# murongshaozong/fabric-token-sdk

Measured on AMD Instinct MI355X. Metric: range-proof verifies/sec (BN254, 64-bit), higher is better.
Workload: dtype u32 (BN254 Fp/Fr 8x32-bit Montgomery); 1 GPU; C2: batch of 4096 standalone 64-bit Bulletproof range proofs per GPU (exact transcripts per proof + RLC batch check via one Pippenger MSM); batch_per_gpu=4096, bit_length=64, rounds=6, parallelism=shard1

## Files before the change

### fabric-token-sdk_amd/csrc/device/fixed_base.hpp

```cpp
#pragma once
#include "g1.hpp"

namespace fts {

constexpr int FB_W = 16;
constexpr int FB_NW = (255 + FB_W - 1) / FB_W;
constexpr int FB_E = 1 << (FB_W - 1);
constexpr size_t FB_WORDS_PER_BASE = (size_t)FB_NW * FB_E * 16;
constexpr int FB_S = 1 << ((FB_W) / 2);
constexpr int FB_L = FB_E / FB_S;

template <int W>
struct FbCfg {
  static constexpr int NW = (255 + W - 1) / W;
  static constexpr int E = 1 << (W - 1);
  static constexpr size_t WORDS_PER_BASE = (size_t)NW * E * 16;
  static constexpr int S = 1 << (W / 2);
  static constexpr int L = E / S;
};
constexpr int FBW_W = 20;
using FbWide = FbCfg<FBW_W>;

FTS_DEV int fb_next_digit(uint32_t s[8], int& carry) {
  int d = (int)(s[0] & (uint32_t)(2 * FB_E - 1)) + carry;
// ... 2 lines not shown
  s[7] >>= FB_W;
  carry = d > FB_E;
  return carry ? d - 2 * FB_E : d;
}

FTS_DEV void madd_inl(G1J& p, const G1A& q) {
  if (f_is_zero(p.z)) {
    p.x = q.x;
    p.y = q.y;
    p.z = f_one<FpP>();
    return;
  }
  Fp z1z1 = fp_sqr(p.z);
  Fp u2 = fp_mul(q.x, z1z1);
  Fp s2 = fp_mul(fp_mul(q.y, p.z), z1z1);
  Fp h = f_sub(u2, p.x);
  Fp rr = f_sub(s2, p.y);
  if (f_is_zero(h)) {
    p = f_is_zero(rr) ? g1j_dbl(p) : g1j_identity();
    return;
  }
  Fp hh = fp_sqr(h);
  Fp i = f_dbl(f_dbl(hh));
  Fp j = fp_mul(h, i);
  rr = f_dbl(rr);
  Fp v = fp_mul(p.x, i);
  Fp x3 = f_sub(f_sub(fp_sqr(rr), j), f_dbl(v));
  Fp y3 = f_sub(fp_mul(rr, f_sub(v, x3)), f_dbl(fp_mul(p.y, j)));
  p.z = f_sub(f_sub(fp_sqr(f_add(p.z, h)), z1z1), hh);
  p.x = x3;
  p.y = y3;
}

FTS_DEV G1A fb_entry(const uint32_t* __restrict__ table, int w, int d) {
  const int ad = d < 0 ? -d : d;
  G1A q = load_g1a(table + ((size_t)w * FB_E + (ad - 1)) * 16);
  if (d < 0) q.y = f_neg(q.y);
  return q;
}

FTS_DEV G1J fb_mul(const uint32_t* __restrict__ table, const Scalar& k) {
  uint32_t s[8];
#pragma unroll
  for (int i = 0; i < 8; i++) s[i] = k.v[i];
  G1J acc = g1j_identity();
  int carry = 0, w = 0, d = 0;
  for (; w < FB_NW; w++) {
    d = fb_next_digit(s, carry);
    if (d != 0) break;
  }
  if (w == FB_NW) return acc;
  G1A cur = fb_entry(table, w, d);
  for (;;) {
    int wn = w + 1, dn = 0;
    for (; wn < FB_NW; wn++) {
      dn = fb_next_digit(s, carry);
      if (dn != 0) break;
    }
    G1A nxt;
    if (wn < FB_NW) nxt = fb_entry(table, wn, dn);
    madd_inl(acc, cur);
    if (wn >= FB_NW) break;
    cur = nxt;
    w = wn;
  }
  return acc;
}

FTS_DEV G1J fb_mul2(const uint32_t* __restrict__ ta, const Scalar& ka, const uint32_t* __restrict__ tb,
                    const Scalar& kb) {
  uint32_t sa[8], sb[8];
#pragma unroll
  for (int i = 0; i < 8; i++) sa[i] = ka.v[i], sb[i] = kb.v[i];
  G1J acc = g1j_identity();
  int ca = 0, cb = 0;
  int da = fb_next_digit(sa, ca), db = fb_next_digit(sb, cb);
  G1A qa, qb;
  if (da != 0) qa = fb_entry(ta, 0, da);
  if (db != 0) qb = fb_entry(tb, 0, db);
  for (int w = 0; w < FB_NW; w++) {
    int dan = 0, dbn = 0;
    G1A na, nb;
    if (w + 1 < FB_NW) {
      dan = fb_next_digit(sa, ca);
      dbn = fb_next_digit(sb, cb);
      if (dan != 0) na = fb_entry(ta, w + 1, dan);
      if (dbn != 0) nb = fb_entry(tb, w + 1, dbn);
    }
    if (da != 0) madd_inl(acc, qa);
    if (db != 0) madd_inl(acc, qb);
    da = dan, db = dbn, qa = na, qb = nb;
  }
  return acc;
}

template <int W>
FTS_DEV int fb_next_digit_w(uint32_t s[8], int& carry) {
  constexpr int E = FbCfg<W>::E;
  int d = (int)(s[0] & (uint32_t)(2 * E - 1)) + carry;
#pragma unroll
  for (int i = 0; i < 7; i++) s[i] = (s[i] >> W) | (s[i + 1] << (32 - W));
  s[7] >>= W;
  carry = d > E;
  return carry ? d - 2 * E : d;
}
template <int W>
FTS_DEV G1A fb_entry_w(const uint32_t* __restrict__ table, int w, int d) {
  const int ad = d < 0 ? -d : d;
  G1A q = load_g1a(table + ((size_t)w * FbCfg<W>::E + (ad - 1)) * 16);
  if (d < 0) q.y = f_neg(q.y);
  return q;
}
template <int W>
FTS_DEV G1J fb_mul_w(const uint32_t* __restrict__ table, const Scalar& k) {
  constexpr int NW = FbCfg<W>::NW;
  uint32_t s[8];
#pragma unroll
  for (int i = 0; i < 8; i++) s[i] = k.v[i];
  G1J acc = g1j_identity();
  int carry = 0, w = 0, d = 0;
  for (; w < NW; w++) {
    d = fb_next_digit_w<W>(s, carry);
    if (d != 0) break;
  }
  if (w == NW) return acc;
  G1A cur = fb_entry_w<W>(table, w, d);
  for (;;) {
    int wn = w + 1, dn = 0;
    for (; wn < NW; wn++) {
      dn = fb_next_digit_w<W>(s, carry);
      if (dn != 0) break;
    }
    G1A nxt;
    if (wn < NW) nxt = fb_entry_w<W>(table, wn, dn);
    madd_inl(acc, cur);
    if (wn >= NW) break;
    cur = nxt;
    w = wn;
  }
  return acc;
}

FTS_DEV void fb_mul_acc(G1J& acc, const uint32_t* __restrict__ table, const Scalar& k) {
  uint32_t s[8];
#pragma unroll
  for (int i = 0; i < 8; i++) s[i] = k.v[i];
  int carry = 0, w = 0, d = 0;
  for (; w < FB_NW; w++) {
    d = fb_next_digit(s, carry);
    if (d != 0) break;
  }
  if (w == FB_NW) return;
  G1A cur = fb_entry(table, w, d);
  for (;;) {
    int wn = w + 1, dn = 0;
    for (; wn < FB_NW; wn++) {
      dn = fb_next_digit(s, carry);
      if (dn != 0) break;
    }
    G1A nxt;
    if (wn < FB_NW) nxt = fb_entry(table, wn, dn);
    madd_inl(acc, cur);
    if (wn >= FB_NW) break;
    cur = nxt;
    w = wn;
  }
}

template <int W>
FTS_DEV void fb_mul_acc_w(G1J& acc, const uint32_t* __restrict__ table, const Scalar& k) {
  constexpr int NW = FbCfg<W>::NW;
  uint32_t s[8];
#pragma unroll
  for (int i = 0; i < 8; i++) s[i] = k.v[i];
  int carry = 0, w = 0, d = 0;
  for (; w < NW; w++) {
    d = fb_next_digit_w<W>(s, carry);
    if (d != 0) break;
  }
  if (w == NW) return;
  G1A cur = fb_entry_w<W>(table, w, d);
  for (;;) {
    int wn = w + 1, dn = 0;
    for (; wn < NW; wn++) {
      dn = fb_next_digit_w<W>(s, carry);
      if (dn != 0) break;
    }
    G1A nxt;
    if (wn < NW) nxt = fb_entry_w<W>(table, wn, dn);
    madd_inl(acc, cur);
    if (wn >= NW) break;
    cur = nxt;
    w = wn;
  }
}

__device__ __noinline__ G1J nl_fb_mul(const uint32_t* __restrict__ table, Scalar k) { return fb_mul(table, k); }

}
```

### fabric-token-sdk_amd/csrc/device/g1.hpp

```cpp
#pragma once
#include "field.hpp"

namespace fts {

struct G1A {
  Fp x, y;
};
struct G1J {
  Fp x, y, z;
};
struct Scalar {
  uint32_t v[8];
};

struct G1J;
__device__ __noinline__ G1J nl_dbl(G1J p);

FTS_DEV Fp fp_mul(const Fp& a, const Fp& b) { return f_mul_g(a, b); }
FTS_DEV Fp fp_sqr(const Fp& a) { return f_mul_g(a, a); }
FTS_DEV Fr fr_mul(const Fr& a, const Fr& b) { return f_mul_g(a, b); }
FTS_DEV Fr fr_sqr(const Fr& a) { return f_mul_g(a, a); }

FTS_DEV G1J g1j_identity() {
  G1J r;
// ... 63 lines not shown
  G1J r;
  r.x = f_sub(f_sub(fp_sqr(rr), j), f_dbl(v));
  r.y = f_sub(fp_mul(rr, f_sub(v, r.x)), f_dbl(fp_mul(p.y, j)));
  r.z = f_sub(f_sub(fp_sqr(f_add(p.z, h)), z1z1), hh);
  return r;
}

FTS_DEV G1J g1j_add(const G1J& p, const G1J& q) {
  if (f_is_zero(p.z)) return q;
  if (f_is_zero(q.z)) return p;
  Fp z1z1 = fp_sqr(p.z);
  Fp z2z2 = fp_sqr(q.z);
  Fp u1 = fp_mul(p.x, z2z2);
  Fp u2 = fp_mul(q.x, z1z1);
  Fp s1 = fp_mul(fp_mul(p.y, q.z), z2z2);
  Fp s2 = fp_mul(fp_mul(q.y, p.z), z1z1);
  Fp h = f_sub(u2, u1);
  Fp rr = f_sub(s2, s1);
  if (f_is_zero(h)) {
    if (f_is_zero(rr)) return nl_dbl(p);
    return g1j_identity();
  }
  Fp i = fp_sqr(f_dbl(h));
  Fp j = fp_mul(h, i);
  rr = f_dbl(rr);
  Fp v = fp_mul(u1, i);
  G1J r;
  r.x = f_sub(f_sub(fp_sqr(rr), j), f_dbl(v));
  r.y = f_sub(fp_mul(rr, f_sub(v, r.x)), f_dbl(fp_mul(s1, j)));
  r.z = fp_mul(f_sub(f_sub(fp_sqr(f_add(p.z, q.z)), z1z1), z2z2), h);
  return r;
}

__device__ __noinline__ Fp nl_fp_inv(Fp a) { return f_inv_gcd(a); }
__device__ __noinline__ Fr nl_fr_inv(Fr a) { return f_inv_gcd(a); }

FTS_DEV bool g1j_eq(const G1J& p, const G1J& q) {
  bool pi = f_is_zero(p.z), qi = f_is_zero(q.z);
  if (pi || qi) return pi && qi;
  Fp z1z1 = fp_sqr(p.z), z2z2 = fp_sqr(q.z);
  if (!f_eq(fp_mul(p.x, z2z2), fp_mul(q.x, z1z1))) return false;
  return f_eq(fp_mul(fp_mul(p.y, q.z), z2z2), fp_mul(fp_mul(q.y, p.z), z1z1));
}

FTS_DEV G1A g1j_to_affine(const G1J& p) {
  G1A r;
  if (f_is_zero(p.z)) {
    r.x = f_zero<FpP>();
    r.y = f_zero<FpP>();
    return r;
  }
  Fp zi = nl_fp_inv(p.z);
  Fp zi2 = fp_sqr(zi);
  r.x = fp_mul(p.x, zi2);
  r.y = fp_mul(fp_mul(p.y, zi2), zi);
  return r;
}

__device__ __noinline__ G1J nl_dbl(G1J p) { return g1j_dbl(p); }

FTS_DEV void load_fp(const uint32_t* src, Fp& a) {
  const uint4* s = reinterpret_cast<const uint4*>(src);
  uint4 u0 = s[0], u1 = s[1];
  a.v[0] = u0.x; a.v[1] = u0.y; a.v[2] = u0.z; a.v[3] = u0.w;
  a.v[4] = u1.x; a.v[5] = u1.y; a.v[6] = u1.z; a.v[7] = u1.w;
}
// ... 102 lines not shown
```

### fabric-token-sdk_amd/csrc/device/glv.hpp

```cpp
#pragma once
#include "fixed_base.hpp"

namespace fts {

struct Glv {
  static constexpr uint32_t BETA[8] = {0xd782e155u, 0x71930c11u, 0xffbe3323u, 0xa6bb947cu,
                                       0xd4741444u, 0xaa303344u, 0x26594943u, 0x2c3b3f0du};
  static constexpr uint32_t G1[7] = {0x2fafba64u, 0x8fa7d32du, 0x773a6ef2u, 0x6eb9c714u,
                                     0xc7e0b3d7u, 0xd91d232eu, 0x00000002u};
  static constexpr uint32_t G2[9] = {0x9b9bdffau, 0x86937516u, 0x5eaa26d9u, 0xa5e38cfbu, 0x391eb18du,
                                     0x7a7bd9d4u, 0xa773d2cfu, 0x4ccef014u, 0x00000002u};
  static constexpr uint32_t A1[2] = {0x94d213e3u, 0x89d32568u};
  static constexpr uint32_t A2[4] = {0x1221250bu, 0x0be4e154u, 0xeeb859fdu, 0x6f4d8248u};
  static constexpr uint32_t NB1[4] = {0x7d4f1128u, 0x8211bbebu, 0xeeb859fcu, 0x6f4d8248u};
};

template <int G>
FTS_DEV void glv_round(const uint32_t k[8], const uint32_t (&g)[G], uint32_t c[5]) {
  uint32_t t[8 + G];
#pragma unroll
  for (int i = 0; i < 8 + G; i++) t[i] = 0;
#pragma unroll
  for (int i = 0; i < 8; i++) {
    uint64_t carry = 0;
// ... 46 lines not shown

template <class K = Glv>
FTS_DEV void glv_decompose(const uint32_t k[8], uint32_t k1[4], uint32_t& s1, uint32_t k2[4], uint32_t& s2) {
  uint32_t c1[5], c2[5];
  glv_round<7>(k, K::G1, c1);
  glv_round<9>(k, K::G2, c2);
  uint32_t r1[8], r2[8];
#pragma unroll
  for (int i = 0; i < 8; i++) {
    r1[i] = k[i];
    r2[i] = 0;
  }
  sub_mul_256<3, 2>(r1, c1, K::A1);
  sub_mul_256<5, 4>(r1, c2, K::A2);
  sub_mul_256<5, 2>(r2, c2, K::A1);
  {
    uint32_t p[8];
#pragma unroll
    for (int i = 0; i < 8; i++) p[i] = 0;
    sub_mul_256<3, 4>(p, c1, K::NB1);
    uint32_t bw = 0;
#pragma unroll
    for (int i = 0; i < 8; i++) r2[i] = subb(r2[i], p[i], bw, bw);
  }
  s1 = glv_abs(r1, k1);
  s2 = glv_abs(r2, k2);
}

FTS_DEV Fp glv_beta() {
  Fp b;
#pragma unroll
  for (int i = 0; i < 8; i++) b.v[i] = Glv::BETA[i];
  return b;
}

FTS_DEV void add_inl(G1J& p, const G1J& q) {
  if (f_is_zero(q.z)) return;
  if (f_is_zero(p.z)) {
    p = q;
    return;
  }
  Fp z1z1 = fp_sqr(p.z);
  Fp z2z2 = fp_sqr(q.z);
  Fp u1 = fp_mul(p.x, z2z2);
  Fp u2 = fp_mul(q.x, z1z1);
  Fp s1 = fp_mul(fp_mul(p.y, q.z), z2z2);
  Fp s2 = fp_mul(fp_mul(q.y, p.z), z1z1);
  Fp h = f_sub(u2, u1);
  Fp rr = f_sub(s2, s1);
  if (f_is_zero(h)) {
    p = f_is_zero(rr) ? g1j_dbl(p) : g1j_identity();
    return;
  }
  Fp i = fp_sqr(f_dbl(h));
  Fp j = fp_mul(h, i);
  rr = f_dbl(rr);
  Fp v = fp_mul(u1, i);
  Fp x3 = f_sub(f_sub(fp_sqr(rr), j), f_dbl(v));
  Fp y3 = f_sub(fp_mul(rr, f_sub(v, x3)), f_dbl(fp_mul(s1, j)));
  p.z = fp_mul(f_sub(f_sub(fp_sqr(f_add(p.z, q.z)), z1z1), z2z2), h);
  p.x = x3;
  p.y = y3;
}

FTS_DEV void vtab_store(uint32_t* __restrict__ tab, size_t stride, size_t idx, int e, const G1J& p) {
#pragma unroll
  for (int i = 0; i < 8; i++) {
    tab[((size_t)(e * 24) + i) * stride + idx] = p.x.v[i];
    tab[((size_t)(e * 24) + 8 + i) * stride + idx] = p.y.v[i];
    tab[((size_t)(e * 24) + 16 + i) * stride + idx] = p.z.v[i];
  }
}
FTS_DEV G1J vtab_load(const uint32_t* __restrict__ tab, size_t stride, size_t idx, int e) {
  G1J p;
#pragma unroll
  for (int i = 0; i < 8; i++) {
    p.x.v[i] = tab[((size_t)(e * 24) + i) * stride + idx];
    p.y.v[i] = tab[((size_t)(e * 24) + 8 + i) * stride + idx];
    p.z.v[i] = tab[((size_t)(e * 24) + 16 + i) * stride + idx];
  }
  return p;
}

FTS_DEV G1J vb128j(const G1J& t, const uint32_t kk[4], uint32_t* __restrict__ tab, size_t stride, size_t idx) {
  if (f_is_zero(t.z)) return g1j_identity();
  {
    vtab_store(tab, stride, idx, 0, t);
    G1J cur = g1j_dbl(t);
    vtab_store(tab, stride, idx, 1, cur);
    for (int e = 2; e < 8; e++) {
      add_inl(cur, t);
      vtab_store(tab, stride, idx, e, cur);
    }
  }
  uint32_t s[4];
// ... 328 lines not shown
```

### fabric-token-sdk_amd/csrc/device/rp_kernels.hpp

```cpp
#pragma once
#include <hip/hip_runtime.h>
#include <stdint.h>
#include "launch.hpp"

namespace fts {

constexpr int RP_PT_T1 = 0, RP_PT_T2 = 1, RP_PT_C = 2, RP_PT_D = 3, RP_PT_V = 4, RP_PT_L = 5;
inline __host__ __device__ int rp_npts(int k) { return 5 + 2 * k; }

constexpr int RP_SC_TAU = 0, RP_SC_DELTA = 1, RP_SC_IP = 2, RP_SC_A = 3, RP_SC_B = 4, RP_NSC = 5;

constexpr int CH_X = 0, CH_X2 = 1, CH_Y = 2, CH_YINV = 3, CH_Z = 4, CH_Z2 = 5, CH_POL = 6, CH_X0 = 7, CH_XJ = 8;
inline __host__ __device__ int rp_nch(int k) { return 8 + 2 * k; }

inline __host__ __device__ int tb_G(int n) { return 2 * n; }
inline __host__ __device__ int tb_H(int n) { return 2 * n + 1; }
inline __host__ __device__ int tb_P(int n) { return 2 * n + 2; }
inline __host__ __device__ int tb_Q(int n) { return 2 * n + 3; }
inline __host__ __device__ int tb_K(int n) { return 2 * n + 4; }
inline __host__ __device__ int tb_ped0(int n) { return 2 * n + 5; }
inline __host__ __device__ int tb_count(int n) { return 2 * n + 6; }

inline __host__ __device__ uint32_t x0_array_len(int n) { return 130u * (2u * n + 2u) - 2u; }
inline __host__ __device__ uint32_t x0_msg_len(int n) { return x0_array_len(n) + 46u; }
inline __host__ __device__ uint32_t x0_slot_bytes(int n) { return ((x0_msg_len(n) + 9u + 63u) / 64u) * 64u; }
inline __host__ __device__ uint32_t x0_const_off(int n) { return 8u + 130u * n; }
inline __host__ __device__ uint32_t x0_const_end(int n) { return 8u + 130u * (2u * n + 1u); }
inline __host__ __device__ uint32_t x0_cb0(int n) { return (x0_const_off(n) + 63u) / 64u; }
inline __host__ __device__ uint32_t x0_cb1(int n) { return x0_const_end(n) / 64u; }
inline __host__ __device__ uint32_t x0_var_bytes(int n) { return x0_slot_bytes(n) - 64u * (x0_cb1(n) - x0_cb0(n)); }

constexpr uint32_t SMALL_SLOT = 512;

constexpr double MADS_PER_MUL = 136.0;
constexpr double COST_MADD = 11.0;
constexpr double COST_ADD = 16.0;
constexpr double COST_DBL = 7.0;
constexpr double COST_INV = 0.0;
constexpr double COST_NORM1 = COST_INV + 4.0;
constexpr double COST_FB = 16.0 * COST_MADD;
constexpr double COST_FB_FRESH = 15.0 * COST_MADD;
constexpr double COST_FBW = 13.0 * COST_MADD;
constexpr double COST_FBW_FRESH = 12.0 * COST_MADD;
constexpr double COST_VB4 = 7.0 + 6.0 * COST_MADD + 256.0 * COST_DBL + 60.0 * COST_ADD;
constexpr double COST_VB128 = 7.0 + 6.0 * COST_ADD + 124.0 * COST_DBL + 30.0 * COST_ADD;
constexpr double COST_STRAUS2 = 2.0 * (7.0 + 6.0 * COST_ADD) + 124.0 * COST_DBL + 60.0 * COST_ADD;
constexpr double COST_STRAUS2_ATAB = (COST_DBL + 6.0 * COST_MADD) + (COST_DBL + 6.0 * COST_ADD) + 109.0 +
                                     124.0 * COST_DBL + 60.0 * COST_MADD;
constexpr double COST_STRAUS2_CTAB = (COST_DBL + 6.0 * COST_ADD) + 61.0 + 124.0 * COST_DBL + 60.0 * COST_MADD;
constexpr double COST_NORM = 7.0;

struct Timeline {
  static constexpr int CAP = 96;
  bool in_fallback = false;
  static constexpr int MAXS = 4;
  hipEvent_t ev[CAP + 1];
  const char* name[CAP];
  double work[CAP];
  int start[CAP];
  int n = 0;
  hipStream_t sl[MAXS];
  int last[MAXS];
  int ns = 0;
  bool created = false;
  void create() {
    if (created) return;
    for (int i = 0; i <= CAP; i++) (void)hipEventCreate(&ev[i]);
    created = true;
  }
  void destroy() {
    if (!created) return;
    for (int i = 0; i <= CAP; i++) (void)hipEventDestroy(ev[i]);
    created = false;
  }
  int& last_of(hipStream_t s) {
    for (int i = 0; i < ns; i++)
// ... 104 lines not shown
```

### fabric-token-sdk_amd/csrc/idemix_identity.hip

```cpp
#include <hip/hip_runtime.h>
#include <stdint.h>
#include <string.h>
#include <sys/random.h>

#include <algorithm>
#include <atomic>
#include <functional>
#include <memory>
#include <mutex>
#include <string>
#include <type_traits>
#include <unordered_map>
#include <vector>

#include "../../include/fts_gpu.h"
#include "common/chacha20.hpp"
#include "common/sha256.hpp"
#include "device/fixed_base.hpp"
#include "device/glv.hpp"
#include "device/helpers.hpp"
#include "device/transcript.hpp"
#include "device/fp256bn.hpp"
#include "device/pairing.hpp"
#include "device/launch.hpp"
// ... 34 lines not shown
  using PJ = G1J;
  static constexpr int G1_BYTES = 64;
  static FTS_DEV PJ inf() { return g1j_identity(); }
  static FTS_DEV bool is_inf(const PJ& p) { return f_is_zero(p.z); }
  static FTS_DEV PJ dbl(const PJ& p) { return g1j_dbl(p); }
  static FTS_DEV void add_to(PJ& acc, const PJ& q) { add_inl(acc, q); }
  static FTS_DEV void madd_to(PJ& acc, const F& x, const F& y) {
    G1A q;
    q.x = x, q.y = y;
    madd_inl(acc, q);
  }
  static FTS_DEV PJ from_affine(const F& x, const F& y) {
    PJ r;
    r.x = x, r.y = y, r.z = f_one<FpP>();
    return r;
  }
  static FTS_DEV bool decode(const uint8_t* raw, F& x, F& y, bool& ident) {
    G1A a;
    const bool ok = decode_point(raw, a);
    ident = ok && g1a_is_identity(a);
    x = a.x, y = a.y;
    return ok;
  }
  template <class Sink>
  static FTS_DEV void encode(Sink& s, const F& x, const F& y) {
    uint32_t pw[16];
    g1_mont_to_be_words(x, y, pw);
    for (int k = 0; k < 16; k++) s.put_word(pw[k]);
  }
  static FTS_DEV void fixed_mul_acc(PJ& acc, const uint32_t* tables, int base, const uint32_t* k) {
    Scalar s;
#pragma unroll
    for (int q = 0; q < 8; q++) s.v[q] = k[q];
    fb_mul_acc(acc, tables + (size_t)base * FB_WORDS_PER_BASE, s);
  }
  static FTS_DEV void decompose(const uint32_t k[8], uint32_t k1[4], uint32_t& s1, uint32_t k2[4], uint32_t& s2) {
    glv_decompose<Glv>(k, k1, s1, k2, s2);
  }
  static FTS_DEV F beta() { return glv_beta(); }
  static FTS_DEV void digest_mod_r(const uint32_t st[8], uint32_t out[8]) {
    const Fr r = digest_to_fr(st);
#pragma unroll
    for (int q = 0; q < 8; q++) out[q] = r.v[q];
  }
};

constexpr int FBN_NW = 16, FBN_ND = 1 << 16;
struct FbnCurve {
  using B = pair::FbnField;
  using F = fbn::Fp;
  using PJ = fbn::PJ;
  static constexpr int G1_BYTES = 65;
  static FTS_DEV PJ inf() { return fbn::pj_inf(); }
  static FTS_DEV bool is_inf(const PJ& p) { return fbn::is_zero(p.z); }
  static FTS_DEV PJ dbl(const PJ& p) { return fbn::pj_dbl(p); }
  static FTS_DEV void add_to(PJ& acc, const PJ& q) { acc = fbn::pj_add(acc, q); }
  static FTS_DEV void madd_to(PJ& acc, const F& x, const F& y) { acc = fbn::pj_madd(acc, x, y); }
  static FTS_DEV PJ from_affine(const F& x, const F& y) {
    PJ r;
    r.x = x, r.y = y, r.z = fbn::load<fbn::PM>(fbn::PM::ONE);
    return r;
  }
  static FTS_DEV bool decode(const uint8_t* raw, F& x, F& y, bool& ident) {
    uint32_t pw[16];
    load_be_words(raw, pw);
    uint32_t nx[8], ny[8];
#pragma unroll
// ... 1340 lines not shown
```

### fabric-token-sdk_amd/csrc/msm.hip

```cpp
#include <algorithm>

#include "device/g1.hpp"
#include "device/glv.hpp"
#include "device/fixed_base.hpp"
#include "device/helpers.hpp"
#include "device/msm.hpp"
#include "device/rp_kernels.hpp"
#include "device/coop.hpp"
#include "device/launch.hpp"

namespace fts {


FTS_DEV uint32_t scalar_bits4(const uint32_t s[4], int off, int width) {
  int q = off >> 5, r = off & 31;
  uint64_t lo = 0, hi = 0;
#pragma unroll
  for (int i = 0; i < 4; i++) {
    if (i == q) lo = s[i];
    if (i == q + 1) hi = s[i];
  }
  uint64_t v = (lo | (hi << 32)) >> r;
  return (uint32_t)(v & ((1ull << width) - 1));
}
// ... 347 lines not shown
    for (uint32_t e = t; e < n; e += blockDim.x) {
      const uint32_t x = tmp[lo + e];
      const uint32_t pos = atomicAdd(&cur[(x >> 24) & (PB - 1)], 1u);
      stage[pos] = (x & RS_IDX_MASK) | (x & 0x80000000u);
    }
    __syncthreads();
    for (uint32_t e = t; e < n; e += blockDim.x) sorted[lo + e] = stage[e];
    return;
  }
  for (uint32_t e = t; e < n; e += blockDim.x) {
    const uint32_t x = tmp[lo + e];
    const uint32_t pos = atomicAdd(&cur[(x >> 24) & (PB - 1)], 1u);
    sorted[lo + pos] = (x & RS_IDX_MASK) | (x & 0x80000000u);
  }
}

__global__ void __launch_bounds__(64, 4) k_msm_chunks(MsmIdx p, const uint32_t* __restrict__ nc_total,
                                                   const MsmWindow* __restrict__ win,
                                                   const uint32_t* __restrict__ points,
                                                   const uint32_t* __restrict__ offsets,
                                                   const uint32_t* __restrict__ counts,
                                                   const uint32_t* __restrict__ chunk_off,
                                                   const int32_t* __restrict__ chunk_bkt,
                                                   const uint32_t* __restrict__ sorted, uint32_t* __restrict__ partials) {
  wave_prio<PS_CHUNKS>();
  const int N = p.N;
  int g = blockIdx.x * blockDim.x + threadIdx.x;
  if (g >= (int)*nc_total) return;
  const int b = chunk_bkt[g];
  const uint32_t j = (uint32_t)g - chunk_off[b], cnt = counts[b];
  const uint32_t lo = j * (uint32_t)p.ch, hi = min(cnt, lo + (uint32_t)p.ch);
  const uint32_t* S = sorted + offsets[b];
  const Fp beta = glv_beta();
  G1J acc = g1j_identity();
  uint32_t e = S[lo];
  G1A q = load_g1a(points + (size_t)msm_src(p, (int)((e & 0x7fffffffu) >= (uint32_t)N ? (e & 0x7fffffffu) - N
                                                                                      : (e & 0x7fffffffu))) * 16);
  for (uint32_t t = lo; t < hi; t++) {
    uint32_t en = 0;
    G1A qn;
    if (t + 1 < hi) {
      en = S[t + 1];
      const uint32_t vn = en & 0x7fffffffu;
      qn = load_g1a(points + (size_t)msm_src(p, (int)(vn >= (uint32_t)N ? vn - N : vn)) * 16);
    }
    if (!g1a_is_identity(q)) {
      if ((e & 0x7fffffffu) >= (uint32_t)N) q.x = fp_mul(q.x, beta);
      if (e >> 31) q.y = f_neg(q.y);
      madd_inl(acc, q);
    }
    e = en;
    q = qn;
  }
  store_g1j(partials + (size_t)g * 24, acc);
}

__global__ void __launch_bounds__(256) k_msm_bucket_sum(int NB, int ch, const uint32_t* __restrict__ counts,
                                                       const uint32_t* __restrict__ chunk_off,
                                                       const uint32_t* __restrict__ partials,
                                                       uint32_t* __restrict__ buckets) {
  wave_prio<PS_MSMTAIL>();
  int b = blockIdx.x * blockDim.x + threadIdx.x;
  if (b >= NB) return;
  const uint32_t nch = (counts[b] + ch - 1) / ch, c0 = chunk_off[b];
  G1J acc = g1j_identity();
  if (nch) acc = load_g1j(partials + (size_t)c0 * 24);
  for (uint32_t q = 1; q < nch; q++) add_inl(acc, load_g1j(partials + (size_t)(c0 + q) * 24));
  store_g1j(buckets + (size_t)b * 24, acc);
}

__global__ void __launch_bounds__(256) k_msm_segments(int nw, int NS, int NSg, int NBg, const MsmWindow* __restrict__ win,
                                                     const uint32_t* __restrict__ buckets,
                                                     uint32_t* __restrict__ segs, uint32_t* __restrict__ scratch) {
  wave_prio<PS_MSMTAIL>();
  int g = blockIdx.x * blockDim.x + threadIdx.x;
  if (g >= NS) return;
  const int grp = g / NSg, gl = g % NSg;
  int w = 0;
  while (w + 1 < nw && win[w + 1].sbase <= gl) w++;
  const MsmWindow W = win[w];
  const int nb = 1 << (W.width - 1);
  const int s = gl - W.sbase;
  const int lo = s * MSM_SEG, cnt = (nb - lo) < MSM_SEG ? (nb - lo) : MSM_SEG;
  const uint32_t* Bk = buckets + ((size_t)grp * NBg + W.bbase + lo) * 24;
  G1J sum = g1j_identity(), acc = g1j_identity();
  for (int j = cnt - 1; j >= 0; j--) {
    add_inl(sum, load_g1j(Bk + j * 24));
// ... 197 lines not shown
    hipLaunchKernelGGL(k_rs_hist, dim3(S), dim3(256), lds, s, ix, spg, npg, p.d_win, hk, hist);
    tl->mark("k_rs_hist", s, 0);
    FTS_LAUNCH(k_rs_pscan, NP, 256, s, p.G, spg, npg, hist, ptot);
    hipLaunchKernelGGL(k_rs_pbase, dim3(1), dim3(RS_PB_BS), 0, s, NP, ptot, pbase);
    tl->mark("k_rs_pscan", s, 0);
    hipLaunchKernelGGL(k_rs_scatter, dim3(S), dim3(256), lds, s, ix, spg, npg, p.d_win, hk, hist, pbase, tmp);
    tl->mark("k_rs_scatter", s, 0);
    hipLaunchKernelGGL(k_rs_part, dim3(NP), dim3(256), 0, s, pbase, ptot, tmp, p.counts, p.sorted);
    tl->mark("k_rs_part", s, 0);
    FTS_LAUNCH(k_msm_scan1, (size_t)p.NBLK * 256, 256, s, p.NB, p.ch, p.counts, p.offsets, p.chunk_off, p.scratch);
    hipLaunchKernelGGL(k_msm_scan2, dim3(1), dim3(256), 0, s, p.NBLK, p.scratch);
    FTS_LAUNCH(k_msm_scan3, p.NB, 256, s, p.NB, p.ch, p.counts, p.offsets, nullptr, p.chunk_off, p.chunk_bkt,
               p.scratch);
    tl->mark("k_msm_scan", s, 0);
  } else {
    (void)hipMemsetAsync(p.counts, 0, (size_t)p.NB * 4, s);
    FTS_LAUNCH(k_msm_digits, p.N, 256, s, msm_idx(p), p.d_win, scalars, p.keys, p.cursor, p.counts);
    tl->mark("k_msm_digits", s, 0);
    FTS_LAUNCH(k_msm_scan1, (size_t)p.NBLK * 256, 256, s, p.NB, p.ch, p.counts, p.offsets, p.chunk_off, p.scratch);
    hipLaunchKernelGGL(k_msm_scan2, dim3(1), dim3(256), 0, s, p.NBLK, p.scratch);
    FTS_LAUNCH(k_msm_scan3, p.NB, 256, s, p.NB, p.ch, p.counts, p.offsets, p.cursor, p.chunk_off, p.chunk_bkt,
               p.scratch);
    tl->mark("k_msm_scan", s, 0);
    FTS_LAUNCH(k_msm_scatter, p.NV, 256, s, p.NV, p.nw, p.keys, p.cursor, p.offsets, p.sorted);
    tl->mark("k_msm_scatter", s, 0);
  }
}

static void launch_msm_accumulate(const MsmPlan& p, const uint32_t* points, hipStream_t s, Timeline* tl,
                                  hipEvent_t ev_stage = nullptr, int stage = 0) {
  FTS_LAUNCH(k_msm_chunks, p.NC, 64, s, msm_idx(p), p.scratch + 2 * (size_t)p.NBLK + 1, p.d_win, points, p.offsets,
             p.counts, p.chunk_off,
             p.chunk_bkt, p.sorted, p.partials);
  tl->mark("k_msm_chunks", s, (double)p.NV * p.nw * (COST_MADD + 0.5));
  if (ev_stage && stage == 2) (void)hipEventRecord(ev_stage, s);
  FTS_LAUNCH(k_msm_bucket_sum, p.NB, g_lat_bs, s, p.NB, p.ch, p.counts, p.chunk_off, p.partials, p.buckets);
  tl->mark("k_msm_bucket_sum", s, 0);
}

static void launch_msm_buckets(const MsmPlan& p, const uint32_t* points, const uint32_t* scalars, hipStream_t s,
                               Timeline* tl, hipEvent_t ev_stage = nullptr, int stage = 0) {
  launch_msm_sort(p, scalars, s, tl);
  if (ev_stage && stage == 1) (void)hipEventRecord(ev_stage, s);
  launch_msm_accumulate(p, points, s, tl, ev_stage, stage);
}

static void launch_msm_tail(const MsmPlan& p, const uint32_t* extra, int nextra, uint32_t* scratch, hipStream_t s,
                            hipStream_t s_extra, Timeline* tl);

void launch_msm_reduce(const MsmPlan& p, const uint32_t* points, const uint32_t* extra, int nextra, uint32_t* scratch,
                       hipStream_t s, hipStream_t s_extra, Timeline* tl) {
  launch_msm_accumulate(p, points, s, tl);
  launch_msm_tail(p, extra, nextra, scratch, s, s_extra, tl);
}

void launch_msm(const MsmPlan& p, const uint32_t* points, const uint32_t* scalars, const uint32_t* extra, int nextra,
                uint32_t* scratch, hipStream_t s, hipStream_t s_extra, Timeline* tl, hipEvent_t ev_stage, int stage) {
  launch_msm_sort(p, scalars, s, tl);
  if (ev_stage && stage == 1) (void)hipEventRecord(ev_stage, s);
  launch_msm_accumulate(p, points, s, tl, ev_stage, stage);
  launch_msm_tail(p, extra, nextra, scratch, s, s_extra, tl);
}

static void launch_msm_tail(const MsmPlan& p, const uint32_t* extra, int nextra, uint32_t* scratch, hipStream_t s,
                            hipStream_t s_extra, Timeline* tl) {
  FTS_LAUNCH(k_msm_segments, p.NS, g_lat_bs, s, p.nw, p.NS, p.NSg, p.NBg, p.d_win, p.buckets, p.segs, scratch);
  tl->mark("k_msm_segments", s, (double)p.NB * 2 * COST_ADD);
// ... 44 lines not shown
```

### fabric-token-sdk_amd/csrc/rp_kernels.hip

```cpp
#include <atomic>
#include "device/g1.hpp"
#include "device/fixed_base.hpp"
#include "device/glv.hpp"
#include "device/rp_kernels.hpp"
#include "device/transcript.hpp"
#include "device/helpers.hpp"
#include "device/msm.hpp"
#include "device/coop.hpp"
#include "device/launch.hpp"
#include "common/chacha20.hpp"
#include "../../include/fts_gpu.h"

namespace fts {
int g_lat_bs = 256;
std::atomic<int> g_work_bs{64};
constexpr int g_chain_bs = 64;


constexpr int NORM_BS = 256;
constexpr int NORM_E = 16;
constexpr size_t NORM_BIG = (size_t)1 << 16;
template <int E>
__global__ void __launch_bounds__(NORM_BS) k_rp_normalize(int total, int per, int stride, int first,
                                                          const int32_t* __restrict__ status,
// ... 1342 lines not shown
  const size_t nbw = (size_t)nb * C::NW;
  return nbw * 24 * 4 + nbw * (C::S + C::L) * 24 * 4 + nbw * C::E * 24 * 4;
}
size_t table_build_scratch_bytes(int nb) { return build_scratch_bytes<FB_W>(nb); }
size_t wide_build_scratch_bytes(int nb, int wbits) {
  return wbits == 22 ? build_scratch_bytes<22>(nb) : build_scratch_bytes<FBW_W>(nb);
}
template <int W>
static void build_tables(const uint32_t* bases, int nb, uint32_t* tables, uint32_t* scratch, hipStream_t s) {
  using C = FbCfg<W>;
  const size_t nbw = (size_t)nb * C::NW;
  uint32_t* bw = scratch;
  uint32_t* small = bw + nbw * 24;
  uint32_t* large = small + nbw * C::S * 24;
  uint32_t* jac = large + nbw * C::L * 24;
  FTS_LAUNCH(kt_window_bases<W>, nbw, 64, s, bases, nb, bw);
  FTS_LAUNCH(kt_small_large<W>, nbw, 64, s, nb, bw, small, large);
  FTS_LAUNCH(kt_entries<W>, nbw * C::E, 64, s, nb, small, large, jac);
  const size_t tot = nbw * C::E;
  launch_normalize(tot, 1, 1, 0, (const int32_t*)nullptr, jac, tables, (uint8_t*)nullptr, s);
}
void launch_build_tables(const uint32_t* bases, int nb, uint32_t* tables, uint32_t* scratch, hipStream_t s) {
  build_tables<FB_W>(bases, nb, tables, scratch, s);
}
void launch_build_wide_tables(const uint32_t* bases, int nb, uint32_t* tables, uint32_t* scratch, hipStream_t s,
                              int wbits) {
  if (wbits == 22) build_tables<22>(bases, nb, tables, scratch, s);
  else build_tables<FBW_W>(bases, nb, tables, scratch, s);
}

void launch_rp_batch(const RpBatchDev& d, const RlcDev& r, const uint32_t* tables, const uint32_t* wtables,
                     const uint8_t* x0_const, const uint8_t* x0_tmpl, hipStream_t s, hipStream_t s2, hipStream_t s3,
                     hipStream_t s4, Timeline* tl, int wbits) {
  const double cost_fbw = wbits == 22 ? 11.0 * COST_MADD : COST_FBW_FRESH;
  const int B = d.B, n = d.n, k = d.k, NC = rlc_ncols(n);
  if (!B) return;
  if (d.excl) (void)hipMemsetAsync(d.excl, 0, (size_t)B * 4, s);
  FTS_LAUNCH(k_rp_decode, B * rp_npts(k), 64, s, B, rp_npts(k), d.raw, d.pts, d.status);
  tl->mark("k_rp_decode", s, 0);
  FTS_LAUNCH(k_rp_hash_small, B * (2 + k), 64, s, B, n, k, d.raw, d.status, d.ch, d.small_msgs);
  tl->mark("k_rp_hash_small", s, 0);
  const int nhp = B * n;
  if (d.com_fixed) {
    tl->fork(s, s2);
    FTS_LAUNCH(k_rp_xd, 2 * B, g_lat_bs, s2, B, n, k, d.status, d.pts, d.small_msgs, d.scratch + (size_t)B * (k + 1) * 8,
               d.terms, com_fx_slots(n), n + 2);
    tl->mark("k_rp_xd", s2, (double)B * 2 * COST_VB128);
  }
  const int lbs = d.com_fixed ? g_lat_bs : g_work_bs.load(std::memory_order_relaxed);
  FTS_LAUNCH(k_rp_chal_fr, B, lbs, s, B, n, k, d.status, d.ch, d.scratch);
  tl->mark("k_rp_chal_fr", s, (double)B * (3 * k + 4 * (k + 1) + 12));
  auto rlc_prep = [&]() {
    tl->fork(s, s3);
    if (d.pre_rlc) d.pre_rlc(d.pre_rlc_arg, s3);
    FTS_LAUNCH(k_rlc_prep, B, lbs, s3, B, n, k, d.status, d.excl, d.ipa_flag, d.sc, d.ch, r.key, r.msc, r.coef);
    tl->mark("k_rlc_prep", s3, (double)B * (3 * k + 33));
    (void)hipEventRecord(d.ev_coef, s3);
  };
  const bool grouped = r.G > 1;
  auto rlc_rest = [&](bool presorted = false) {
    auto msm = [&](const uint32_t* extra, int nextra) {
      if (presorted) launch_msm_reduce(r.plan, d.pts, extra, nextra, r.msm_scratch, s3, s4, tl);
      else launch_msm(r.plan, d.pts, r.msc, extra, nextra, r.msm_scratch, s3, s4, tl);
    };
    tl->fork(s, s4);
    tl->fork(s3, s4);
    if (grouped) {
// ... 157 lines not shown

void launch_rp_gather(const RpGather& g, int k, uint8_t* raw, uint32_t* sc, int32_t* status, int32_t* ipa, hipStream_t s) {
  const int per = rp_npts(k) * 4 + RP_NSC * 2 + 1;
  FTS_LAUNCH(k_rp_gather, (size_t)g.off[g.G] * per, 64, s, g, rp_npts(k), raw, sc, status, ipa);
}

void launch_rp_fallback(const RpBatchDev& d, const uint32_t* tables, const int32_t* sel, int nsel, hipStream_t s,
                        Timeline* tl) {
  const int B = sel ? nsel : d.B, n = d.n, k = d.k;
  FTS_LAUNCH(k_rp_terms_fixed, B * (3 + 2 * n), 64, s, B, n, k, sel, d.status, d.ipa_flag, d.sc, d.ch, tables, d.terms);
  tl->mark("k_rp_terms_fixed", s, (double)B * (3 + 2 * n) * COST_FB_FRESH);
  const size_t nvar = (size_t)B * (3 + 2 * k);
  if (nvar <= TV_COOP_MAX)
    FTS_LAUNCH(k_rp_terms_var_coop, (nvar + TV_GPW - 1) / TV_GPW * 64, 64, s, B, n, k, sel, d.status, d.ipa_flag, d.pts,
               d.ch, d.terms);
  else
    FTS_LAUNCH(k_rp_terms_var, nvar, 64, s, B, n, k, sel, d.status, d.ipa_flag, d.pts, d.ch, d.terms, d.scratch);
  tl->mark("k_rp_terms_var", s, (double)B * (3 + 2 * k) * (4.0 * 7.0 + 12.0 * COST_ADD + 124 * COST_DBL + 60 * COST_ADD));
  if (B > 0)
    hipLaunchKernelGGL(k_rp_check, dim3((B + CK_PROOFS - 1) / CK_PROOFS), dim3(CK_LANES * CK_PROOFS), 0, s, B, n, k,
                       sel, d.status, d.ipa_flag, d.terms, d.hpa);
  tl->mark("k_rp_check", s, (double)B * rp_nterms(n, k) * COST_ADD);
}

void launch_rlc_group_test(const RpBatchDev& d, const RlcDev& r, const uint32_t* tables, const MsmPlan& p,
                           const int32_t* sel, int G, int gs, uint32_t* gcol, uint32_t* gfix, int32_t* next,
                           uint32_t* next_count, hipStream_t s, Timeline* tl) {
  const int n = d.n, k = d.k;
  const int NC = rlc_ncols(n);
  if (gs <= GT_SMALL_MAX) {
    const int nch = gt_nchunks(n);
    FTS_LAUNCH(k_rlc_group_cols_small, (size_t)G * nch, 256, s, d.B, n, k, G, gs, sel, d.ch, r.coef, d.ypow, d.svec,
               d.zvec, tables, gfix);
    tl->mark("k_rlc_group_cols", s, (double)G * (gs * 3.0 * n + NC * FB_NW * COST_MADD));
    launch_msm_small(p, d.pts, r.msc, gfix, nch, s, tl);
    FTS_LAUNCH(k_rlc_group_final, (size_t)G * gs, 256, s, G * gs, gs, sel, p.out, d.status, d.ipa_flag, next,
               next_count);
    tl->mark("k_rlc_group_final", s, 0);
    return;
  }
  hipLaunchKernelGGL(k_rlc_columns, dim3(NC, G), dim3(gs <= 64 ? 64 : 256), 0, s, d.B, n, k, gs, 0, sel, d.ch,
                     r.coef, d.ypow, d.svec, d.zvec, gcol);
  tl->mark("k_rlc_group_columns", s, (double)G * gs * 4 * n);
  FTS_LAUNCH(k_rlc_fixed, (size_t)NC * G * FB_NW, RF_ITEMS * FB_NW, s, n, G, 0, NC, gcol, tables, gfix);
  tl->mark("k_rlc_group_fixed", s, (double)G * NC * (FB_NW * 3 + (FB_NW - 1) * COST_ADD));
  launch_msm(p, d.pts, r.msc, gfix, NC, r.msm_scratch, s, s, tl);
  FTS_LAUNCH(k_rlc_group_final, (size_t)G * gs, 256, s, G * gs, gs, sel, p.out, d.status, d.ipa_flag, next,
             next_count);
  tl->mark("k_rlc_group_final", s, 0);
}

}

namespace fts {
__global__ void __launch_bounds__(256) k_msm_gen_points(int N, const uint8_t* __restrict__ raw_k,
                                                       const uint8_t* __restrict__ raw_s,
                                                       const uint32_t* __restrict__ table, uint32_t* __restrict__ jac,
                                                       uint32_t* __restrict__ sc) {
  const int i = blockIdx.x * blockDim.x + threadIdx.x;
  if (i >= N) return;
  auto be_fr = [](const uint8_t* p) {
    uint32_t w[8];
    const uint4* s4 = reinterpret_cast<const uint4*>(p);
#pragma unroll
    for (int q = 0; q < 2; q++) {
      const uint4 u = s4[q];
      w[4 * q + 0] = __builtin_bswap32(u.x);
// ... 29 lines not shown
```

Measured before the change: 5.165 million verifies/s.

## Use extended Jacobian (XYZZ) coordinates for fixed-base and MSM bucket accumulation

Adds an XYZZ point type with mixed-add, full-add and doubling, and switches fixed-base scalar multiplication, fb_mul2 and the MSM chunk accumulation from Jacobian mixed-add to XYZZ mixed-add. Results convert back to Jacobian at the end, and fb_mul_acc now builds a fresh sum and adds it to the accumulator with a full Jacobian add. The aim is fewer field multiplications per mixed addition in the hot accumulation loops. The cost is an extra coordinate per accumulator (more registers) plus a final conversion and, for accumulate variants, an extra full addition. A Jacobian-accumulate variant is kept for the idemix path.

```diff
diff --git a/fabric-token-sdk_amd/csrc/device/fixed_base.hpp b/fabric-token-sdk_amd/csrc/device/fixed_base.hpp
--- a/fabric-token-sdk_amd/csrc/device/fixed_base.hpp
+++ b/fabric-token-sdk_amd/csrc/device/fixed_base.hpp
@@ -58,6 +58,89 @@
   p.y = y3;
 }
 
+FTS_DEV void add_inl(G1J& p, const G1J& q) {
+  if (f_is_zero(q.z)) return;
+  if (f_is_zero(p.z)) {
+    p = q;
+    return;
+  }
+  Fp z1z1 = fp_sqr(p.z);
+  Fp z2z2 = fp_sqr(q.z);
+  Fp u1 = fp_mul(p.x, z2z2);
+  Fp u2 = fp_mul(q.x, z1z1);
+  Fp s1 = fp_mul(fp_mul(p.y, q.z), z2z2);
+  Fp s2 = fp_mul(fp_mul(q.y, p.z), z1z1);
+  Fp h = f_sub(u2, u1);
+  Fp rr = f_sub(s2, s1);
+  if (f_is_zero(h)) {
+    p = f_is_zero(rr) ? g1j_dbl(p) : g1j_identity();
+    return;
+  }
+  Fp i = fp_sqr(f_dbl(h));
+  Fp j = fp_mul(h, i);
+  rr = f_dbl(rr);
+  Fp v = fp_mul(u1, i);
+  Fp x3 = f_sub(f_sub(fp_sqr(rr), j), f_dbl(v));
+  Fp y3 = f_sub(fp_mul(rr, f_sub(v, x3)), f_dbl(fp_mul(s1, j)));
+  p.z = fp_mul(f_sub(f_sub(fp_sqr(f_add(p.z, q.z)), z1z1), z2z2), h);
+  p.x = x3;
+  p.y = y3;
+}
+
+FTS_DEV void xmadd_inl(G1X& p, const G1A& q) {
+  if (f_is_zero(p.zz)) {
+    p.x = q.x;
+    p.y = q.y;
+    p.zz = f_one<FpP>();
+    p.zzz = f_one<FpP>();
+    return;
+  }
+  Fp u2 = fp_mul(q.x, p.zz);
+  Fp s2 = fp_mul(q.y, p.zzz);
+  Fp h = f_sub(u2, p.x);
+  Fp rr = f_sub(s2, p.y);
+  if (f_is_zero(h)) {
+    p = f_is_zero(rr) ? g1x_dbl(p) : g1x_identity();
+    return;
+  }
+  Fp hh = fp_sqr(h);
+  Fp hhh = fp_mul(h, hh);
+  Fp v = fp_mul(p.x, hh);
+  Fp x3 = f_sub(f_sub(fp_sqr(rr), hhh), f_dbl(v));
+  Fp y3 = f_sub(fp_mul(rr, f_sub(v, x3)), fp_mul(p.y, hhh));
+  p.zz = fp_mul(p.zz, hh);
+  p.zzz = fp_mul(p.zzz, hhh);
+  p.x = x3;
+  p.y = y3;
+}
+
+FTS_DEV void xadd_inl(G1X& p, const G1X& q) {
+  if (f_is_zero(q.zz)) return;
+  if (f_is_zero(p.zz)) {
+    p = q;
+    return;
+  }
+  Fp u1 = fp_mul(p.x, q.zz);
+  Fp u2 = fp_mul(q.x, p.zz);
+  Fp s1 = fp_mul(p.y, q.zzz);
+  Fp s2 = fp_mul(q.y, p.zzz);
+  Fp h = f_sub(u2, u1);
+  Fp rr = f_sub(s2, s1);
+  if (f_is_zero(h)) {
+    p = f_is_zero(rr) ? g1x_dbl(p) : g1x_identity();
+    return;
+  }
+  Fp hh = fp_sqr(h);
+  Fp hhh = fp_mul(h, hh);
+  Fp v = fp_mul(u1, hh);
+  Fp x3 = f_sub(f_sub(fp_sqr(rr), hhh), f_dbl(v));
+  Fp y3 = f_sub(fp_mul(rr, f_sub(v, x3)), fp_mul(s1, hhh));
+  p.zz = fp_mul(fp_mul(p.zz, q.zz), hh);
+  p.zzz = fp_mul(fp_mul(p.zzz, q.zzz), hhh);
+  p.x = x3;
+  p.y = y3;
+}
+
 FTS_DEV G1A fb_entry(const uint32_t* __restrict__ table, int w, int d) {
   const int ad = d < 0 ? -d : d;
   G1A q = load_g1a(table + ((size_t)w * FB_E + (ad - 1)) * 16);
@@ -65,40 +148,12 @@
   return q;
 }
 
-FTS_DEV G1J fb_mul(const uint32_t* __restrict__ table, const Scalar& k) {
-  uint32_t s[8];
-#pragma unroll
-  for (int i = 0; i < 8; i++) s[i] = k.v[i];
-  G1J acc = g1j_identity();
-  int carry = 0, w = 0, d = 0;
-  for (; w < FB_NW; w++) {
-    d = fb_next_digit(s, carry);
-    if (d != 0) break;
-  }
-  if (w == FB_NW) return acc;
-  G1A cur = fb_entry(table, w, d);
-  for (;;) {
-    int wn = w + 1, dn = 0;
-    for (; wn < FB_NW; wn++) {
-      dn = fb_next_digit(s, carry);
-      if (dn != 0) break;
-    }
-    G1A nxt;
-    if (wn < FB_NW) nxt = fb_entry(table, wn, dn);
-    madd_inl(acc, cur);
-    if (wn >= FB_NW) break;
-    cur = nxt;
-    w = wn;
-  }
-  return acc;
-}
-
 FTS_DEV G1J fb_mul2(const uint32_t* __restrict__ ta, const Scalar& ka, const uint32_t* __restrict__ tb,
                     const Scalar& kb) {
   uint32_t sa[8], sb[8];
 #pragma unroll
   for (int i = 0; i < 8; i++) sa[i] = ka.v[i], sb[i] = kb.v[i];
-  G1J acc = g1j_identity();
+  G1X acc = g1x_identity();
   int ca = 0, cb = 0;
   int da = fb_next_digit(sa, ca), db = fb_next_digit(sb, cb);
   G1A qa, qb;
@@ -113,11 +168,11 @@
       if (dan != 0) na = fb_entry(ta, w + 1, dan);
       if (dbn != 0) nb = fb_entry(tb, w + 1, dbn);
     }
-    if (da != 0) madd_inl(acc, qa);
-    if (db != 0) madd_inl(acc, qb);
+    if (da != 0) xmadd_inl(acc, qa);
+    if (db != 0) xmadd_inl(acc, qb);
     da = dan, db = dbn, qa = na, qb = nb;
   }
-  return acc;
+  return g1x_to_jac(acc);
 }
 
 template <int W>
@@ -138,12 +193,12 @@
   return q;
 }
 template <int W>
-FTS_DEV G1J fb_mul_w(const uint32_t* __restrict__ table, const Scalar& k) {
+FTS_DEV G1X fb_sum_w(const uint32_t* __restrict__ table, const Scalar& k) {
   constexpr int NW = FbCfg<W>::NW;
   uint32_t s[8];
 #pragma unroll
   for (int i = 0; i < 8; i++) s[i] = k.v[i];
-  G1J acc = g1j_identity();
+  G1X acc = g1x_identity();
   int carry = 0, w = 0, d = 0;
   for (; w < NW; w++) {
     d = fb_next_digit_w<W>(s, carry);
@@ -159,15 +214,29 @@
     }
     G1A nxt;
     if (wn < NW) nxt = fb_entry_w<W>(table, wn, dn);
-    madd_inl(acc, cur);
+    xmadd_inl(acc, cur);
     if (wn >= NW) break;
     cur = nxt;
     w = wn;
   }
   return acc;
 }
-
+template <int W>
+FTS_DEV G1J fb_mul_w(const uint32_t* __restrict__ table, const Scalar& k) {
+  return g1x_to_jac(fb_sum_w<W>(table, k));
+}
+
+template <int W>
+FTS_DEV void fb_mul_acc_w(G1J& acc, const uint32_t* __restrict__ table, const Scalar& k) {
+  const G1X s = fb_sum_w<W>(table, k);
+  if (f_is_zero(s.zz)) return;
+  add_inl(acc, g1x_to_jac(s));
+}
 FTS_DEV void fb_mul_acc(G1J& acc, const uint32_t* __restrict__ table, const Scalar& k) {
+  fb_mul_acc_w<FB_W>(acc, table, k);
+}
+
+FTS_DEV void fb_mul_acc_jac(G1J& acc, const uint32_t* __restrict__ table, const Scalar& k) {
   uint32_t s[8];
 #pragma unroll
   for (int i = 0; i < 8; i++) s[i] = k.v[i];
@@ -193,33 +262,7 @@
   }
 }
 
-template <int W>
-FTS_DEV void fb_mul_acc_w(G1J& acc, const uint32_t* __restrict__ table, const Scalar& k) {
-  constexpr int NW = FbCfg<W>::NW;
-  uint32_t s[8];
-#pragma unroll
-  for (int i = 0; i < 8; i++) s[i] = k.v[i];
-  int carry = 0, w = 0, d = 0;
-  for (; w < NW; w++) {
-    d = fb_next_digit_w<W>(s, carry);
-    if (d != 0) break;
-  }
-  if (w == NW) return;
-  G1A cur = fb_entry_w<W>(table, w, d);
-  for (;;) {
-    int wn = w + 1, dn = 0;
-    for (; wn < NW; wn++) {
-      dn = fb_next_digit_w<W>(s, carry);
-      if (dn != 0) break;
-    }
-    G1A nxt;
-    if (wn < NW) nxt = fb_entry_w<W>(table, wn, dn);
-    madd_inl(acc, cur);
-    if (wn >= NW) break;
-    cur = nxt;
-    w = wn;
-  }
-}
+FTS_DEV G1J fb_mul(const uint32_t* __restrict__ table, const Scalar& k) { return fb_mul_w<FB_W>(table, k); }
 
 __device__ __noinline__ G1J nl_fb_mul(const uint32_t* __restrict__ table, Scalar k) { return fb_mul(table, k); }
 
diff --git a/fabric-token-sdk_amd/csrc/device/g1.hpp b/fabric-token-sdk_amd/csrc/device/g1.hpp
--- a/fabric-token-sdk_amd/csrc/device/g1.hpp
+++ b/fabric-token-sdk_amd/csrc/device/g1.hpp
@@ -119,6 +119,39 @@
   return r;
 }
 
+struct G1X {
+  Fp x, y, zz, zzz;
+};
+FTS_DEV G1X g1x_identity() {
+  G1X r;
+  r.x = f_one<FpP>();
+  r.y = f_one<FpP>();
+  r.zz = f_zero<FpP>();
+  r.zzz = f_zero<FpP>();
+  return r;
+}
+FTS_DEV G1J g1x_to_jac(const G1X& p) {
+  G1J r;
+  r.x = fp_mul(p.x, p.zz);
+  r.y = fp_mul(p.y, p.zzz);
+  r.z = p.zz;
+  return r;
+}
+FTS_DEV G1X g1x_dbl(const G1X& p) {
+  Fp u = f_dbl(p.y);
+  Fp v = fp_sqr(u);
+  Fp w = fp_mul(u, v);
+  Fp s = fp_mul(p.x, v);
+  Fp xx = fp_sqr(p.x);
+  Fp m = f_add(f_dbl(xx), xx);
+  G1X r;
+  r.x = f_sub(fp_sqr(m), f_dbl(s));
+  r.y = f_sub(fp_mul(m, f_sub(s, r.x)), fp_mul(w, p.y));
+  r.zz = fp_mul(v, p.zz);
+  r.zzz = fp_mul(w, p.zzz);
+  return r;
+}
+
 __device__ __noinline__ Fp nl_fp_inv(Fp a) { return f_inv_gcd(a); }
 __device__ __noinline__ Fr nl_fr_inv(Fr a) { return f_inv_gcd(a); }
 
diff --git a/fabric-token-sdk_amd/csrc/device/glv.hpp b/fabric-token-sdk_amd/csrc/device/glv.hpp
--- a/fabric-token-sdk_amd/csrc/device/glv.hpp
+++ b/fabric-token-sdk_amd/csrc/device/glv.hpp
@@ -102,35 +102,6 @@
 #pragma unroll
   for (int i = 0; i < 8; i++) b.v[i] = Glv::BETA[i];
   return b;
-}
-
-FTS_DEV void add_inl(G1J& p, const G1J& q) {
-  if (f_is_zero(q.z)) return;
-  if (f_is_zero(p.z)) {
-    p = q;
-    return;
-  }
-  Fp z1z1 = fp_sqr(p.z);
-  Fp z2z2 = fp_sqr(q.z);
-  Fp u1 = fp_mul(p.x, z2z2);
-  Fp u2 = fp_mul(q.x, z1z1);
-  Fp s1 = fp_mul(fp_mul(p.y, q.z), z2z2);
-  Fp s2 = fp_mul(fp_mul(q.y, p.z), z1z1);
-  Fp h = f_sub(u2, u1);
-  Fp rr = f_sub(s2, s1);
-  if (f_is_zero(h)) {
-    p = f_is_zero(rr) ? g1j_dbl(p) : g1j_identity();
-    return;
-  }
-  Fp i = fp_sqr(f_dbl(h));
-  Fp j = fp_mul(h, i);
-  rr = f_dbl(rr);
-  Fp v = fp_mul(u1, i);
-  Fp x3 = f_sub(f_sub(fp_sqr(rr), j), f_dbl(v));
-  Fp y3 = f_sub(fp_mul(rr, f_sub(v, x3)), f_dbl(fp_mul(s1, j)));
-  p.z = fp_mul(f_sub(f_sub(fp_sqr(f_add(p.z, q.z)), z1z1), z2z2), h);
-  p.x = x3;
-  p.y = y3;
 }
 
 FTS_DEV void vtab_store(uint32_t* __restrict__ tab, size_t stride, size_t idx, int e, const G1J& p) {
diff --git a/fabric-token-sdk_amd/csrc/device/rp_kernels.hpp b/fabric-token-sdk_amd/csrc/device/rp_kernels.hpp
--- a/fabric-token-sdk_amd/csrc/device/rp_kernels.hpp
+++ b/fabric-token-sdk_amd/csrc/device/rp_kernels.hpp
@@ -36,12 +36,15 @@
 constexpr double COST_MADD = 11.0;
 constexpr double COST_ADD = 16.0;
 constexpr double COST_DBL = 7.0;
+constexpr double COST_XMADD = 10.0;
+constexpr double COST_XADD = 14.0;
+constexpr double COST_X2J = 2.0;
 constexpr double COST_INV = 0.0;
 constexpr double COST_NORM1 = COST_INV + 4.0;
-constexpr double COST_FB = 16.0 * COST_MADD;
-constexpr double COST_FB_FRESH = 15.0 * COST_MADD;
-constexpr double COST_FBW = 13.0 * COST_MADD;
-constexpr double COST_FBW_FRESH = 12.0 * COST_MADD;
+constexpr double COST_FB_FRESH = 15.0 * COST_XMADD + COST_X2J;
+constexpr double COST_FB = COST_FB_FRESH + COST_ADD;
+constexpr double COST_FBW_FRESH = 12.0 * COST_XMADD + COST_X2J;
+constexpr double COST_FBW = COST_FBW_FRESH + COST_ADD;
 constexpr double COST_VB4 = 7.0 + 6.0 * COST_MADD + 256.0 * COST_DBL + 60.0 * COST_ADD;
 constexpr double COST_VB128 = 7.0 + 6.0 * COST_ADD + 124.0 * COST_DBL + 30.0 * COST_ADD;
 constexpr double COST_STRAUS2 = 2.0 * (7.0 + 6.0 * COST_ADD) + 124.0 * COST_DBL + 60.0 * COST_ADD;
diff --git a/fabric-token-sdk_amd/csrc/idemix_identity.hip b/fabric-token-sdk_amd/csrc/idemix_identity.hip
--- a/fabric-token-sdk_amd/csrc/idemix_identity.hip
+++ b/fabric-token-sdk_amd/csrc/idemix_identity.hip
@@ -90,7 +90,7 @@
     Scalar s;
 #pragma unroll
     for (int q = 0; q < 8; q++) s.v[q] = k[q];
-    fb_mul_acc(acc, tables + (size_t)base * FB_WORDS_PER_BASE, s);
+    fb_mul_acc_jac(acc, tables + (size_t)base * FB_WORDS_PER_BASE, s);
   }
   static FTS_DEV void decompose(const uint32_t k[8], uint32_t k1[4], uint32_t& s1, uint32_t k2[4], uint32_t& s2) {
     glv_decompose<Glv>(k, k1, s1, k2, s2);
diff --git a/fabric-token-sdk_amd/csrc/msm.hip b/fabric-token-sdk_amd/csrc/msm.hip
--- a/fabric-token-sdk_amd/csrc/msm.hip
+++ b/fabric-token-sdk_amd/csrc/msm.hip
@@ -403,7 +403,7 @@
   const uint32_t lo = j * (uint32_t)p.ch, hi = min(cnt, lo + (uint32_t)p.ch);
   const uint32_t* S = sorted + offsets[b];
   const Fp beta = glv_beta();
-  G1J acc = g1j_identity();
+  G1X acc = g1x_identity();
   uint32_t e = S[lo];
   G1A q = load_g1a(points + (size_t)msm_src(p, (int)((e & 0x7fffffffu) >= (uint32_t)N ? (e & 0x7fffffffu) - N
                                                                                       : (e & 0x7fffffffu))) * 16);
@@ -418,12 +418,12 @@
     if (!g1a_is_identity(q)) {
       if ((e & 0x7fffffffu) >= (uint32_t)N) q.x = fp_mul(q.x, beta);
       if (e >> 31) q.y = f_neg(q.y);
-      madd_inl(acc, q);
+      xmadd_inl(acc, q);
     }
     e = en;
     q = qn;
   }
-  store_g1j(partials + (size_t)g * 24, acc);
+  store_g1j(partials + (size_t)g * 24, g1x_to_jac(acc));
 }
 
 __global__ void __launch_bounds__(256) k_msm_bucket_sum(int NB, int ch, const uint32_t* __restrict__ counts,
@@ -687,7 +687,7 @@
   FTS_LAUNCH(k_msm_chunks, p.NC, 64, s, msm_idx(p), p.scratch + 2 * (size_t)p.NBLK + 1, p.d_win, points, p.offsets,
              p.counts, p.chunk_off,
              p.chunk_bkt, p.sorted, p.partials);
-  tl->mark("k_msm_chunks", s, (double)p.NV * p.nw * (COST_MADD + 0.5));
+  tl->mark("k_msm_chunks", s, (double)p.NV * p.nw * (COST_XMADD + 0.5 + COST_X2J / p.ch));
   if (ev_stage && stage == 2) (void)hipEventRecord(ev_stage, s);
   FTS_LAUNCH(k_msm_bucket_sum, p.NB, g_lat_bs, s, p.NB, p.ch, p.counts, p.chunk_off, p.partials, p.buckets);
   tl->mark("k_msm_bucket_sum", s, 0);
diff --git a/fabric-token-sdk_amd/csrc/rp_kernels.hip b/fabric-token-sdk_amd/csrc/rp_kernels.hip
--- a/fabric-token-sdk_amd/csrc/rp_kernels.hip
+++ b/fabric-token-sdk_amd/csrc/rp_kernels.hip
@@ -1398,7 +1398,7 @@
 void launch_rp_batch(const RpBatchDev& d, const RlcDev& r, const uint32_t* tables, const uint32_t* wtables,
                      const uint8_t* x0_const, const uint8_t* x0_tmpl, hipStream_t s, hipStream_t s2, hipStream_t s3,
                      hipStream_t s4, Timeline* tl, int wbits) {
-  const double cost_fbw = wbits == 22 ? 11.0 * COST_MADD : COST_FBW_FRESH;
+  const double cost_fbw = wbits == 22 ? 11.0 * COST_XMADD + COST_X2J : COST_FBW_FRESH;
   const int B = d.B, n = d.n, k = d.k, NC = rlc_ncols(n);
   if (!B) return;
   if (d.excl) (void)hipMemsetAsync(d.excl, 0, (size_t)B * 4, s);
@@ -1622,7 +1622,7 @@
     const int nch = gt_nchunks(n);
     FTS_LAUNCH(k_rlc_group_cols_small, (size_t)G * nch, 256, s, d.B, n, k, G, gs, sel, d.ch, r.coef, d.ypow, d.svec,
                d.zvec, tables, gfix);
-    tl->mark("k_rlc_group_cols", s, (double)G * (gs * 3.0 * n + NC * FB_NW * COST_MADD));
+    tl->mark("k_rlc_group_cols", s, (double)G * (gs * 3.0 * n + NC * COST_FB_FRESH + (NC - nch) * COST_ADD));
     launch_msm_small(p, d.pts, r.msc, gfix, nch, s, tl);
     FTS_LAUNCH(k_rlc_group_final, (size_t)G * gs, 256, s, G * gs, gs, sel, p.out, d.status, d.ipa_flag, next,
                next_count);
```

Measured after the change: 5.386 million verifies/s, median of 6. 4.3% higher.
